# CHEBSB/PolarDecoding

Hardware: AMD Instinct MI355X
Metric: decoded frames/sec, N=1024 K=512 CA-SCL L=8 (higher is better)
Workload: dtype f64

## Files before the change

polardecoding_amd/csrc/scl_fast2.h:

```cpp
#pragma once
#include "fast2_lds.h"
#include "octet_bits.h"
#include "scl_fast.h"

namespace polar {

template <typename R>
struct Fast2Cfg {
    static constexpr int NLOG = 10, N = 1024, NW = 32, TOP = 9, HI = 8, L = 8;
    static constexpr int NA = 32;
    static constexpr int WAVES = 4;
    static constexpr int MIN_WAVES_PER_SIMD = sizeof(R) == 8 ? 3 : 4;
    static constexpr int NFA = HI - 3;
    static constexpr size_t sc_l8 = 0;
    static constexpr size_t sc_l7 = sc_l8 + 8 * 256;
    static constexpr size_t sc_l6 = sc_l7 + 8 * 128;
    static constexpr size_t sc_tl = sc_l6 + 8 * 64;
    static constexpr size_t scratch_cw = sc_tl + 512;
    static constexpr size_t scratch_elems = 2 * scratch_cw;
    static constexpr size_t off_lut = 0;
    static constexpr size_t off_frz = off_lut + ((Lut<R>::bytes + 15) / 16) * 16;
    static constexpr size_t off_msk = off_frz + 4 * NW;
    static constexpr size_t off_kth = off_msk + 4 * CRC_MASK_ROWS * NW;
    static constexpr size_t off_stair = off_kth + 256 * 8;
    static constexpr size_t shared_bytes = off_stair + ((Stair<R>::bytes + 15) / 16) * 16;
    static constexpr size_t off_bl = 0;
    static constexpr size_t off_cw = off_bl + 4 * fast2_lds::ROWS_WORDS;
    static constexpr size_t off_cd = off_cw + 4 * fast2_lds::ROWS_WORDS;
    static constexpr size_t off_ky = off_cd + sizeof(R) * 32;
    static constexpr size_t off_sg = off_ky + 128;
    static constexpr size_t per_wave = off_sg + sizeof(R) * 512;
    static constexpr size_t total = shared_bytes + WAVES * per_wave;
    static_assert(off_cw % 16 == 0 && off_cd % 16 == 0 && per_wave % 16 == 0 && shared_bytes % 16 == 0, "LDS regions are 16-byte aligned");
};
static_assert(3 * Fast2Cfg<double>::total <= 163840 && 4 * Fast2Cfg<float>::total <= 163840, "the pair kernel's LDS limits its occupancy");

template <int QP>
__device__ __forceinline__ double quadp(double x) { return quad_lanes<QP>(x); }
template <int QP>
__device__ __forceinline__ float quadp(float x) { return quad_lanes<QP>(x); }

template <bool FROM_Y>
struct Fast2Sigma { double sigma; };
template <>
struct Fast2Sigma<false> {};

template <typename R, typename IN, bool CRC_ON, bool FROM_Y>
struct Fast2Dec : Fast2Sigma<FROM_Y> {
    using C = Fast2Cfg<R>;
    static constexpr int N = C::N, NW = C::NW, TOP = C::TOP, HI = C::HI, L = 8, NFA = C::NFA;

    R A[C::NA];
    R a1;
    R bp_s, bp_d, bp_ts, bp_td;
    R PM;
    uint32_t ptr, bl0, fl;
    int logact;
    int p, c, pos, lane, gl;
    int own_addr, oth_addr;
    uint32_t pos0_mask;
    int cand_addr;
    Lut<R> lut;
    R *cand, *stg;
    uint32_t *blw, *curw, *keys;
    const unsigned char *kth;
    __amdgpu_buffer_rsrc_t rs_scr;
    __amdgpu_buffer_rsrc_t rs_in;
    unsigned cscr;
    unsigned csrc;
    static __device__ __forceinline__ __amdgpu_buffer_rsrc_t make_rsrc(const void *base, unsigned bytes)
    {
        return __builtin_amdgcn_make_buffer_rsrc(const_cast<void *>(base), 0, (int)bytes, 0x00020000);
    }
    typedef unsigned u2_t __attribute__((ext_vector_type(2)));
    static __device__ __forceinline__ double ld_buf(__amdgpu_buffer_rsrc_t r, unsigned eoff, double, int aux)
    {
        return aux ? __builtin_bit_cast(double, __builtin_amdgcn_raw_buffer_load_b64(r, eoff * 8u, 0, 16))
                   : __builtin_bit_cast(double, __builtin_amdgcn_raw_buffer_load_b64(r, eoff * 8u, 0, 0));
    }
    static __device__ __forceinline__ float ld_buf(__amdgpu_buffer_rsrc_t r, unsigned eoff, float, int aux)
    {
        return aux ? __builtin_bit_cast(float, __builtin_amdgcn_raw_buffer_load_b32(r, eoff * 4u, 0, 16))
                   : __builtin_bit_cast(float, __builtin_amdgcn_raw_buffer_load_b32(r, eoff * 4u, 0, 0));
    }
    static __device__ __forceinline__ void st_buf(__amdgpu_buffer_rsrc_t r, unsigned eoff, double v)
    {
        __builtin_amdgcn_raw_buffer_store_b64(__builtin_bit_cast(u2_t, v), r, eoff * 8u, 0, 0);
    }
    static __device__ __forceinline__ void st_buf(__amdgpu_buffer_rsrc_t r, unsigned eoff, float v)
    {
        __builtin_amdgcn_raw_buffer_store_b32(__builtin_bit_cast(unsigned, v), r, eoff * 4u, 0, 0);
    }
    struct SPtr {
        const Fast2Dec *d;
        unsigned off;
        struct Ref {
            const Fast2Dec *d;
            unsigned off;
            __device__ __forceinline__ void operator=(R v) const { st_buf(d->rs_scr, off, v); }
        };
        __device__ __forceinline__ SPtr operator+(int k) const { return SPtr{d, off + (unsigned)k}; }
        __device__ __forceinline__ Ref operator[](int k) const { return Ref{d, off + (unsigned)k}; }
    };
    static __device__ __forceinline__ R ld_sc(SPtr q) { return ld_buf(q.d->rs_scr, q.off, R(0), 1); }

    static __device__ __forceinline__ int row(int slot) { return fast2_lds::row(slot); }
    __device__ __forceinline__ int pa(int t) const { return (ptr >> (3 * (t - 4))) & 7; }
    __device__ __forceinline__ void set_pa(int t, int v) { ptr = (ptr & ~(7u << (3 * (t - 4)))) | ((uint32_t)v << (3 * (t - 4))); }
    __device__ __forceinline__ int pb(int t) const { return (ptr >> (3 * (NFA + t - 5))) & 7; }
    __device__ __forceinline__ void set_pb(int t, int v) { ptr = (ptr & ~(7u << (3 * (NFA + t - 5)))) | ((uint32_t)v << (3 * (NFA + t - 5))); }
    __device__ __forceinline__ R chk(R a, R b) const { return chk_lut1<R>(a, b, lut); }
    __device__ __forceinline__ R chks(R a, R b) const { return chk_lut1<R>(a, b, lut); }
    __device__ __forceinline__ R chv(int e) const
    {
        double v = (double)ld_buf(rs_in, csrc + (unsigned)e, IN(0), 0);
        if constexpr (FROM_Y) v = llr_from_y(v, this->sigma);
        return (R)v;
    }
    static __device__ __forceinline__ unsigned fresh(unsigned off)
    {
        __asm__ volatile("" : "+v"(off));
        return off;
    }
    __device__ __forceinline__ SPtr l8(int slot) const { return SPtr{this, fresh(cscr + (unsigned)(C::sc_l8 + slot * 256))}; }
    __device__ __forceinline__ SPtr l7(int slot) const { return SPtr{this, fresh(cscr + (unsigned)(C::sc_l7 + slot * 128))}; }
    __device__ __forceinline__ SPtr tls() const { return SPtr{this, fresh(cscr + (unsigned)C::sc_tl)}; }

    template <int T>
    __device__ __forceinline__ void f_reg()
    {
        constexpr int RO = (1 << T) / 4;
#pragma unroll
        for (int r = 0; r < RO; ++r) A[RO + r] = chk(A[2 * RO + r], A[3 * RO + r]);
        if constexpr (T >= 4) set_pa(T, p);
    }
    template <int T>
    __device__ __forceinline__ void g_reg()
    {
        constexpr int RO = (1 << T) / 4;
        const int sl = pa(T + 1) * 8 + gl;
        uint32_t w;
        if constexpr (T == 5) w = blw[row(pb(5)) + 1] >> pos;
        else w = bl0 >> (16 + pos);
#pragma unroll
        for (int r = 0; r < RO; ++r) {
            const R x = __shfl(A[2 * RO + r], sl), y = __shfl(A[3 * RO + r], sl);
            A[RO + r] = g_bit<R>(x, y, w, 4 * r);
        }
        set_pa(T, p);
    }
    __device__ __forceinline__ void g3()
    {
        const int sl = pa(4) * 8 + gl;
        const uint32_t w = bl0 >> (8 + pos);
#pragma unroll
        for (int r = 0; r < 2; ++r) {
            const R x = __shfl(A[4 + r], sl), y = __shfl(A[6 + r], sl);
            A[2 + r] = g_bit<R>(x, y, w, 4 * r);
        }
    }

    __device__ __forceinline__ void push_l6(R v)
    {
#pragma unroll
        for (int r = 16; r < 31; ++r) A[r] = A[r + 1];
        A[31] = v;
    }
    __device__ __forceinline__ void load_l6() { set_pa(6, p); }
    __device__ __forceinline__ R top_src(bool right, int idx, int q) const
    {
        const int seg = idx >> 4, within = idx & 15;
        const int e = 16 * q + within + 64 * (seg & 3) + 256 * (seg >> 2);
        return right ? chv(e) : ld_sc(tls() + e);
    }
    __device__ __forceinline__ void from_top(bool right, bool gstep)
    {
        vm_drain();
        const uint32_t *bt = blw + row(pb(TOP)) + 16;
        const uint32_t *bh = blw + row(pb(HI)) + 8;
        const SPtr o8 = l8(p), o7 = l7(p);
        const int w32 = (int)fresh((unsigned)(p * 4 + pos));
        const int nld = right ? 8 : 4;
        R *pre = A + 4;
#pragma unroll
        for (int m = 0; m < 8; ++m) pre[m] = (m < nld) ? top_src(right, w32 + 32 * m, 0) : R(0);
        for (int q = 0; q < 4; ++q) {
            lds_fence();
#pragma unroll
            for (int m = 0; m < 8; ++m)
                if (m < nld) stg[w32 + 32 * m] = pre[m];
            lds_fence();
            if (q < 3) {
#pragma unroll
                for (int m = 0; m < 8; ++m) pre[m] = (m < nld) ? top_src(right, w32 + 32 * m, q + 1) : R(0);
            }
#pragma unroll 1
            for (int i = 0; i < 4; ++i) {
                const int rr = 4 * q + i;
                const int e0 = pos + 4 * rr;
                const int sh = 4 * (rr & 7);
                const int wq = rr >> 3;
                const int wi = 4 * i + pos;
                R *v8 = A + 12;
#pragma unroll
                for (int k = 0; k < 4; ++k) {
                    const int e = e0 + 64 * k;
                    R x, y;
                    if (right) {
                        const uint32_t w0 = bt[2 * k + wq] >> pos, w1 = bt[8 + 2 * k + wq] >> pos;
                        x = g_bit<R>(stg[(k + 0) * 16 + wi], stg[(k + 8) * 16 + wi], w0, sh);
                        y = g_bit<R>(stg[(k + 4) * 16 + wi], stg[(k + 12) * 16 + wi], w1, sh);
                    } else {
                        x = stg[(k + 0) * 16 + wi];
                        y = stg[(k + 4) * 16 + wi];
                    }
                    if (gstep) v8[k] = g_bit<R>(x, y, bh[2 * k + wq] >> pos, sh);
                    else v8[k] = chk(x, y);
                    o8[e] = v8[k];
                }
                const R v70 = chk(v8[0], v8[2]), v71 = chk(v8[1], v8[3]);
                o7[e0] = v70;
                o7[e0 + 64] = v71;
                push_l6(chk(v70, v71));
            }
        }
        set_pa(8, p);
        set_pa(7, p);
        load_l6();
    }
    __device__ __forceinline__ void from_l8()
    {
        vm_drain();
        const SPtr s8 = l8(pa(8));
        const uint32_t *b7 = blw + row(pb(7)) + 4;
        const SPtr o7 = l7(p);
        constexpr int CP = sizeof(R) == 8 ? 2 : 4;
        for (int q = 0; q < 16 / CP; ++q) {
            R *in = A;
#pragma unroll
            for (int i = 0; i < CP; ++i) {
                const int e0 = pos + 4 * (CP * q + i);
#pragma unroll
                for (int k = 0; k < 4; ++k) in[4 * i + k] = ld_sc(s8 + e0 + 64 * k);
            }
#pragma unroll
            for (int i = 0; i < CP; ++i) {
                const int rr = CP * q + i;
                const int e0 = pos + 4 * rr;
                const int sh = 4 * (rr & 7);
                const int wq = rr >> 3;
                const R v70 = g_bit<R>(in[4 * i], in[4 * i + 2], b7[wq] >> pos, sh);
                const R v71 = g_bit<R>(in[4 * i + 1], in[4 * i + 3], b7[2 + wq] >> pos, sh);
                o7[e0] = v70;
                o7[e0 + 64] = v71;
                push_l6(chk(v70, v71));
            }
        }
        set_pa(7, p);
        load_l6();
    }
    __device__ __forceinline__ void from_l7()
    {
        vm_drain();
        const SPtr s7 = l7(pa(7)) + pos;
        const uint32_t *b6 = blw + row(pb(6)) + 2;
        const uint32_t w0 = b6[0] >> pos, w1 = b6[1] >> pos;
#pragma unroll
        for (int r = 0; r < 16; ++r) {
            const R x = ld_sc(s7 + 4 * r), y = ld_sc(s7 + 4 * r + 64);
            A[16 + r] = g_bit<R>(x, y, r < 8 ? w0 : w1, 4 * (r & 7));
        }
        set_pa(6, p);
    }

    __device__ __forceinline__ void octet_head(int o)
    {
        const int d = (o == 0) ? 10 : 3 + __builtin_ctz((unsigned)o);
        if (d >= 8) from_top(o >= N / 16, d == 8);
        else if (d == 7) from_l8();
        else if (d == 6) from_l7();
        else if (d == 5) g_reg<5>();
        else if (d == 4) g_reg<4>();
        else g3();
        if (d > 5) f_reg<5>();
        if (d > 4) f_reg<4>();
        if (d > 3) f_reg<3>();
    }
    __device__ __forceinline__ void octet_head_reg(int o)
    {
        const int d = 3 + __builtin_ctz((unsigned)o);
        if (d == 5) g_reg<5>();
        else if (d == 4) g_reg<4>();
        else g3();
        if (d > 4) f_reg<4>();
        if (d > 3) f_reg<3>();
    }

    template <int K>
    __device__ __forceinline__ void set_bit_k(int o, uint32_t bit)
    {
        if constexpr (K < 7) {
            bl0 |= bit << K;
        } else {
            const uint32_t c3 = octet_bits::level3((bl0 & 0x7Fu) | (bit << 7));
            bl0 &= ~0xFFu;
            set_bit7(o, c3);
        }
    }
    __device__ __forceinline__ void set_bit7(int o, uint32_t c3)
    {
        if ((o & 1) == 0) {
            bl0 = (bl0 & ~0xFF00u) | (c3 << 8);
            return;
        }
        const uint32_t c4 = (((bl0 >> 8) & 0xFFu) ^ c3) | (c3 << 8);
        if ((o & 2) == 0) {
            bl0 = (bl0 & 0xFFFFu) | (c4 << 16);
            return;
        }
        set_bit_lds(8 * o + 7, ((bl0 >> 16) ^ c4) | (c4 << 16));
    }
    __device__ __forceinline__ void set_bit_lds(int j, uint32_t cur)
    {
        const int own = (int)fresh((unsigned)row(p));
        lds_fence();
        if (pos == 0) curw[own] = cur;
        lds_fence();
        int t = 5;
        while (t < 10 && ((j >> t) & 1)) {
            const int nw = 1 << (t - 5);
            const int sb = pb(t);
            for (int w = pos; w < nw; w += 4) {
                const uint32_t cc = curw[own + w];
                const uint32_t l = blw[row(sb) + nw + w];
                curw[own + w] = l ^ cc;
                curw[own + w + nw] = cc;
            }
            lds_fence();
            ++t;
        }
        if (t < 10) {
            const int nw = 1 << (t - 5);
            for (int w = pos; w < nw; w += 4) blw[own + nw + w] = curw[own + w];
            set_pb(t, p);
            lds_fence();
        }
    }

    __device__ __forceinline__ uint32_t survivors(R c0, R c1)
    {
        lds_fence();
        if (pos == 0) {
            keys[2 * p] = metric_key(c0);
            keys[2 * p + 1] = metric_key(c1);
        }
        lds_fence();
        const unsigned char *kb = reinterpret_cast<const unsigned char *>(keys) - 64 * c;
        const uint32_t own = *reinterpret_cast<const uint32_t *>(kb + own_addr);
        const uint32_t oth = *reinterpret_cast<const uint32_t *>(kb + oth_addr);
        const uint32_t own1 = own + 1u;
        uint32_t acc = (oth - own1) >> 31;
        acc = __builtin_amdgcn_alignbit(acc, (uint32_t)dpp_i<0x121>((int)oth) - own1, 31);
        acc = __builtin_amdgcn_alignbit(acc, (uint32_t)dpp_i<0x122>((int)oth) - own1, 31);
        acc = __builtin_amdgcn_alignbit(acc, (uint32_t)dpp_i<0x123>((int)oth) - own1, 31);
        acc = __builtin_amdgcn_alignbit(acc, (uint32_t)dpp_i<0x124>((int)oth) - own1, 31);
        acc = __builtin_amdgcn_alignbit(acc, (uint32_t)dpp_i<0x125>((int)oth) - own1, 31);
        acc = __builtin_amdgcn_alignbit(acc, (uint32_t)dpp_i<0x126>((int)oth) - own1, 31);
        acc = __builtin_amdgcn_alignbit(acc, (uint32_t)dpp_i<0x127>((int)oth) - own1, 31);
        uint32_t cnt = __popc(acc);
        {
            auto r = __builtin_amdgcn_permlane16_swap(cnt, cnt, false, false);
            cnt = r[0] + r[1];
        }
        uint64_t b = __ballot(cnt <= (uint32_t)L);
        uint32_t m_a = (uint32_t)b & 0xFFFFu, m_b = (uint32_t)(b >> 32) & 0xFFFFu;
        if (sizeof(R) == 8 && (__popc(m_a) != L || __popc(m_b) != L)) {
            if (__popc(c ? m_b : m_a) != L) fl |= 0x4u;
            lds_fence();
            if (pos == 0) {
                cand[p] = c0;
                cand[8 + p] = c1;
            }
            lds_fence();
            const R *cb = reinterpret_cast<const R *>(reinterpret_cast<const unsigned char *>(cand) - (int)sizeof(R) * 16 * c);
            const R *mycand = reinterpret_cast<const R *>(reinterpret_cast<const unsigned char *>(cb) + cand_addr);
            const R mine = mycand[lane & 15];
            int n = 0;
#pragma unroll
            for (int m = 0; m < 16; ++m) n += (mycand[m] <= mine) ? 1 : 0;
            b = __ballot(n <= L);
            m_a = (uint32_t)b & 0xFFFFu;
            m_b = (uint32_t)(b >> 32) & 0xFFFFu;
        }
        return c ? m_b : m_a;
    }

    __device__ __forceinline__ bool trivial_prune(R cb, R cw) const
    {
        uint32_t mx = metric_key(cb) & pos0_mask;
        mx = max(mx, (uint32_t)dpp_i<0x128>((int)mx));
        {
            auto a = __builtin_amdgcn_permlane16_swap(mx, mx, false, false);
            mx = max(a[0], a[1]);
        }
        {
            auto a = __builtin_amdgcn_permlane32_swap(mx, mx, false, false);
            mx = max(a[0], a[1]);
        }
        return __ballot(mx >= (metric_key(cw) | ~pos0_mask)) == 0ull;
    }
    static __device__ __forceinline__ uint32_t sign_bit(double x) { return (uint32_t)__double2hiint(x) >> 31; }
    static __device__ __forceinline__ uint32_t sign_bit(float x) { return (uint32_t)__float_as_int(x) >> 31; }

    template <int K, bool FULL>
    __device__ __forceinline__ void decide(int o, bool frozen, R lam) { decide_t<K, FULL>(o, frozen, lam, lut.tabv(lam)); }
    template <int K, bool FULL>
    __device__ __forceinline__ void decide_t(int o, bool frozen, R lam, R tt)
    {
        if (frozen) {
            PM += tt + negmax(lam);
            set_bit_k<K>(o, 0u);
            return;
        }
        uint32_t bit;
        R pm;
        if (!FULL && logact < 3) {
            const R ph0 = tt + negmax(lam), ph1 = tt + posmax(lam);
            bit = (p >> logact) & 1;
            pm = PM + (bit ? ph1 : ph0);
            ++logact;
        } else {
            const uint32_t lneg = sign_bit(lam);
            const R cb = PM + tt, cw = PM + (tt + absr(lam));
            bit = (uint32_t)dpp_i<0x00>((int)lneg);
            pm = cb;
            if (!trivial_prune(cb, cw)) ranked<K>(lneg, cb, cw, bit, pm);
        }
        PM = pm;
        set_bit_k<K>(o, bit);
    }
    template <int K>
    __device__ __forceinline__ void ranked(uint32_t lneg, R cb, R cw, uint32_t &bit, R &pm)
    {
        const R c0 = lneg ? cw : cb, c1 = lneg ? cb : cw;
        const uint32_t mask = survivors(c0, c1);
        const uint32_t m0 = mask & 0xFFu, m1 = mask >> 8;
        const uint32_t m_both = m0 & m1, m_dead = ~(m0 | m1) & 0xFFu;
        if (__popc(mask) < L) fl |= 0x1u;
        const bool s0 = (m0 >> p) & 1, s1 = (m1 >> p) & 1;
        bit = (!s0 && s1) ? 1u : 0u;
        pm = bit ? c1 : c0;
        if (__ballot(m_dead != 0u) == 0ull) return;
        const bool dead = !s0 && !s1;
        const int myrank = __popc(m_dead & ((1u << p) - 1u));
        const bool refilled = dead && (myrank < __popc(m_both));
        const int src = (int)kth[m_both * 8 + myrank];
        const int sg = refilled ? src : p;
        const int sl = sg * 8 + gl;
        const R c1s = __shfl(c1, sl);
        ptr = __shfl(ptr, sl);
        bl0 = __shfl(bl0, sl);
        if constexpr ((K & 4) == 0) { A[2] = __shfl(A[2], sl); A[3] = __shfl(A[3], sl); }
        if constexpr ((K & 2) == 0) { A[1] = __shfl(A[1], sl); a1 = __shfl(a1, sl); }
        if constexpr ((K & 1) == 0) { bp_d = __shfl(bp_d, sl); bp_td = __shfl(bp_td, sl); }
        bit = refilled ? 1u : bit;
        pm = refilled ? c1s : pm;
    }

    __device__ __forceinline__ void frozen_prefix(int P, int nphi, bool regs, R &xl, R &yl)
    {
        const int w32 = p * 4 + pos, j0 = 8 * P;
        vm_drain();
        {
            const SPtr tl = tls();
            const SPtr o8 = l8(0), o7 = l7(0);
            R v8[8];
#pragma unroll
            for (int k = 0; k < 8; ++k) {
                const int e = w32 + 32 * k;
                v8[k] = chk(ld_sc(tl + e), ld_sc(tl + e + 256));
                o8[e] = v8[k];
            }
            lds_fence();
#pragma unroll
            for (int k = 0; k < 4; ++k) {
                const R v7 = chk(v8[k], v8[k + 4]);
                o7[w32 + 32 * k] = v7;
                stg[w32 + 32 * k] = v7;
            }
            set_pa(8, 0);
            set_pa(7, 0);
        }
        lds_fence();
#pragma unroll
        for (int t = 6; t >= 0; --t) {
            const int h = 1 << t;
            int idx[2];
            R x[2], y[2];
#pragma unroll
            for (int i = 0; i < 2; ++i) {
                const int b = w32 + 32 * i;
                idx[i] = ((b >> t) << (t + 1)) | (b & (h - 1));
                x[i] = stg[idx[i]];
                y[i] = stg[idx[i] + h];
            }
            if (t == 0) {
                xl = stg[126];
                yl = stg[127];
            }
            lds_fence();
#pragma unroll
            for (int i = 0; i < 2; ++i) {
                stg[idx[i]] = chk(x[i], y[i]);
                stg[idx[i] + h] = y[i] + x[i];
            }
            lds_fence();
            if (t >= 4 && regs) {
                const R *node = stg + ((j0 >> t) << t) + pos;
#pragma unroll
                for (int r = 0; r < h / 4; ++r) A[h / 4 + r] = node[4 * r];
            }
        }
#pragma unroll
        for (int k = 0; k < 4; ++k) {
            const R lam = stg[w32 + 32 * k];
            stg[128 + w32 + 32 * k] = lut.tabv(lam) + negmax(lam);
        }
        lds_fence();
        R pm = PM;
#pragma unroll 8
        for (int j = 0; j < nphi; ++j) pm += stg[128 + j];
        PM = pm;
        lds_fence();
    }

    __device__ __forceinline__ uint32_t fill_tail(uint32_t f2, R lam0, R xl, R yl)
    {
        uint32_t b0 = 0, b1 = 0;
        if (!(f2 & 1u)) {
            b0 = (p >> logact) & 1;
            ++logact;
        }
        PM += lut.tabv(lam0) + (b0 ? posmax(lam0) : negmax(lam0));
        const R lam1 = b0 ? -(xl - yl) : yl + xl;
        if (!(f2 & 2u)) {
            b1 = (p >> logact) & 1;
            ++logact;
        }
        PM += lut.tabv(lam1) + (b1 ? posmax(lam1) : negmax(lam1));
        return (b0 ? 0x55555555u : 0u) ^ (b1 ? 0xFFFFFFFFu : 0u);
    }
    __device__ __forceinline__ void fill_phase(int E, const uint32_t *frz, R xl, R yl)
    {
        const int w32 = (int)fresh((unsigned)(p * 4 + pos));
        const int qb = (p & 1) * 64;
        const uint32_t wv0 = fill_tail(frz[3] >> 30, stg[126], xl, yl);
        uint32_t wv1 = 0;
        lds_fence();
        blw[row(p) + 4 + pos] = wv0;
        lds_fence();
#pragma unroll 1
        for (int S = 128; S < E; S += 64) {
            vm_drain();
            const uint32_t wsel = S == 128 ? wv0 : wv1;
            uint32_t wq[2];
            wq[0] = (uint32_t)__shfl((int)wsel, gl) >> w32;
            wq[1] = (uint32_t)__shfl((int)wsel, 8 + gl) >> w32;
            if (S == 128) {
                const SPtr s8 = l8(0) + w32;
                R v8[8];
#pragma unroll
                for (int k = 0; k < 8; ++k) v8[k] = ld_sc(s8 + 32 * k);
#pragma unroll
                for (int q = 0; q < 2; ++q) {
                    const SPtr o7 = l7(q) + w32;
                    R v7[4];
#pragma unroll
                    for (int k = 0; k < 4; ++k) {
                        v7[k] = g_bit<R>(v8[k], v8[k + 4], wq[q], 0);
                        o7[32 * k] = v7[k];
                    }
                    stg[64 * q + w32] = chk(v7[0], v7[2]);
                    stg[64 * q + w32 + 32] = chk(v7[1], v7[3]);
                }
                set_pa(7, p & 1);
            } else {
#pragma unroll
                for (int q = 0; q < 2; ++q) {
                    const SPtr s7 = l7(q) + w32;
#pragma unroll
                    for (int i = 0; i < 2; ++i)
                        stg[64 * q + w32 + 32 * i] = g_bit<R>(ld_sc(s7 + 32 * i), ld_sc(s7 + 32 * i + 64), wq[q], 0);
                }
            }
            lds_fence();
#pragma unroll
            for (int t = 5; t >= 0; --t) {
                const int h = 1 << t;
                int idx[2];
                R x[2], y[2];
#pragma unroll
                for (int i = 0; i < 2; ++i) {
                    const int b = w32 + 32 * i;
                    idx[i] = ((b >> t) << (t + 1)) | (b & (h - 1));
                    x[i] = stg[idx[i]];
                    y[i] = stg[idx[i] + h];
                }
                if (t == 0) {
                    xl = stg[qb + 62];
                    yl = stg[qb + 63];
                }
                lds_fence();
#pragma unroll
                for (int i = 0; i < 2; ++i) {
                    stg[idx[i]] = chk(x[i], y[i]);
                    stg[idx[i] + h] = y[i] + x[i];
                }
                lds_fence();
            }
#pragma unroll
            for (int k = 0; k < 4; ++k) {
                const R lam = stg[w32 + 32 * k];
                stg[128 + w32 + 32 * k] = lut.tabv(lam) + negmax(lam);
            }
            lds_fence();
            R pm = PM;
#pragma unroll 2
            for (int j = 0; j < 62; ++j) pm += stg[128 + qb + j];
            PM = pm;
            const uint32_t wv = fill_tail(frz[(S + 62) >> 5] >> 30, stg[qb + 62], xl, yl);
            lds_fence();
            if (S == 128) {
                wv1 = wv;
                if (pos < 2) blw[row(p) + 2 + pos] = wv;
            } else {
                const uint32_t b = pos < 2 ? wv1 ^ wv : wv;
                blw[row(p) + 8 + pos] = wv0 ^ b;
                blw[row(p) + 12 + pos] = b;
            }
            lds_fence();
        }
    }

    template <bool FULL>
    __device__ __forceinline__ void octet_frozen_prefix(int o, bool last_frozen)
    {
        R xf = chks(A[2], A[3]), xg = A[3] + A[2];
        R yf = quadp<0x4E>(xf), yg = quadp<0x4E>(xg);
        {
            const R ff = chks(xf, yf), gf = xf + yf, fg = chks(xg, yg), gg = xg + yg;
            xf = (pos & 2) ? gf : ff;
            xg = (pos & 2) ? gg : fg;
        }
        yf = quadp<0xB1>(xf); yg = quadp<0xB1>(xg);
        R lf, lg;
        {
            const R ff = chks(xf, yf), gf = xf + yf, fg = chks(xg, yg), gg = xg + yg;
            lf = (pos & 1) ? gf : ff;
            lg = (pos & 1) ? gg : fg;
        }
        const R pf = lut.tabv(lf) + negmax(lf), pg = lut.tabv(lg) + negmax(lg);
        PM += pf;
        PM += quadp<0x55>(pf);
        PM += quadp<0xAA>(pf);
        PM += quadp<0xFF>(pf);
        PM += pg;
        PM += quadp<0x55>(pg);
        PM += quadp<0xAA>(pg);
        if (last_frozen) {
            PM += quadp<0xFF>(pg);
            set_bit7(o, 0u);
        } else {
            decide<7, FULL>(o, false, quadp<0xFF>(lg));
        }
    }

    struct ChkBp { R v, s, d, ts, td; };
    __device__ __forceinline__ ChkBp chk_bp(R x, R y) const
    {
        ChkBp r;
        r.s = x + y;
        r.d = x - y;
        r.ts = lut.tabv(r.s);
        r.td = lut.tabv(r.d);
        r.v = xor_sign(minabs(x, y), x, y) + (r.ts - r.td);
        return r;
    }
    static __device__ __forceinline__ R g_sel(R sum, R dif, uint32_t w, int sh)
    {
        const uint32_t m = (uint32_t)__builtin_amdgcn_sbfe((int)w, sh, 1);
        return Lut<R>::sel_mask(m, -dif, sum);
    }
    template <int K, bool FULL>
    __device__ __forceinline__ void leaf_pair(int o, uint32_t fm, R x1)
    {
        const ChkBp q = chk_bp(x1, quadp<0xB1>(x1));
        bp_d = q.d;
        bp_td = q.td;
        decide<K, FULL>(o, (fm >> K) & 1, q.v);
        const uint32_t m1 = (uint32_t)__builtin_amdgcn_sbfe((int)bl0, K, 1);
        decide_t<K + 1, FULL>(o, (fm >> (K + 1)) & 1, Lut<R>::sel_mask(m1, -bp_d, q.s), Lut<R>::sel_mask(m1, bp_td, q.ts));
    }
    template <bool FULL>
    __device__ __forceinline__ void octet(int o, uint32_t fm)
    {
        {
            const R s2 = A[2] + A[3], d2 = A[2] - A[3];
            const R v2 = xor_sign(minabs(A[2], A[3]), A[2], A[3]) + (lut.tabv(s2) - lut.tabv(d2));
            A[2] = s2;
            A[3] = d2;
            const R y2 = quadp<0x4E>(v2);
            const R s1 = v2 + y2, d1 = v2 - y2;
            const R v1 = xor_sign(minabs(v2, y2), v2, y2) + (lut.tabv(s1) - lut.tabv(d1));
            A[1] = s1;
            a1 = d1;
            leaf_pair<0, FULL>(o, fm, v1);
        }
        leaf_pair<2, FULL>(o, fm, g_sel(A[1], a1, octet_bits::level1_lo(bl0), pos));
        {
            const R v2 = g_sel(A[2], A[3], octet_bits::level2(bl0), pos);
            const R y2 = quadp<0x4E>(v2);
            const R s1 = v2 + y2, d1 = v2 - y2;
            const R v1 = xor_sign(minabs(v2, y2), v2, y2) + (lut.tabv(s1) - lut.tabv(d1));
            A[1] = s1;
            a1 = d1;
            leaf_pair<4, FULL>(o, fm, v1);
        }
        leaf_pair<6, FULL>(o, fm, g_sel(A[1], a1, octet_bits::level1_hi(bl0), pos));
    }
};

template <typename D, bool FULL>
__device__ __forceinline__ int octet_group(D &s, const uint32_t *frz, uint32_t &fword, int o)
{
    s.octet_head(o);
    for (;;) {
        if ((o & 3) == 0) fword = frz[o >> 2];
        const uint32_t fm = (fword >> (8 * (o & 3))) & 0xFFu;
        if ((fm & 0x7Fu) != 0x7Fu) s.template octet<FULL>(o, fm);
        else s.template octet_frozen_prefix<FULL>(o, fm == 0xFFu);
        ++o;
        if ((o & 7) == 0) break;
        s.octet_head_reg(o);
    }
    return o;
}

template <typename R, typename IN, bool CRC_ON, bool FROM_Y>
__device__ __forceinline__ void scl_fast2_body(const SclParams &P)
{
    using D = Fast2Dec<R, IN, CRC_ON, FROM_Y>;
    using C = Fast2Cfg<R>;
    constexpr int N = C::N, NW = C::NW, L = 8;
    extern __shared__ __attribute__((aligned(16))) unsigned char smem[];
    const int wave = __builtin_amdgcn_readfirstlane(threadIdx.x >> 6);
    unsigned char *base = smem + C::shared_bytes + (size_t)wave * C::per_wave;
    uint32_t *frz = reinterpret_cast<uint32_t *>(smem + C::off_frz);
    uint32_t *msk = reinterpret_cast<uint32_t *>(smem + C::off_msk);
    unsigned char *kth = smem + C::off_kth;

    Lut<R>::build(smem + C::off_lut, threadIdx.x, blockDim.x);
    for (int i = threadIdx.x; i < NW; i += blockDim.x) frz[i] = P.frozen[i];
    if (CRC_ON)
        for (int i = threadIdx.x; i < CRC_MASK_ROWS * NW; i += blockDim.x)
            msk[i] = P.crc_mask[(i & ~(NW - 1)) + ((i >> 3) & 3) + 4 * (i & 7)];
    for (int i = threadIdx.x; i < 256 * 8; i += blockDim.x) {
        int m = i >> 3, k = i & 7, idx = 0, seen = 0;
        for (int b = 0; b < 8; ++b)
            if ((m >> b) & 1) {
                if (seen == k) idx = b;
                ++seen;
            }
        kth[i] = (unsigned char)idx;
    }
    __syncthreads();

    D s;
    s.lane = threadIdx.x & 63;
    s.p = s.lane >> 3;
    s.c = (s.lane >> 2) & 1;
    s.pos = s.lane & 3;
    s.pos0_mask = s.pos == 0 ? 0xFFFFFFFFu : 0u;
    s.gl = s.lane & 7;
    s.lut.bind(smem + C::off_lut);
    s.kth = kth;
    s.blw = reinterpret_cast<uint32_t *>(base + C::off_bl) + fast2_lds::cw_base(1) * s.c;
    s.curw = reinterpret_cast<uint32_t *>(base + C::off_cw) + fast2_lds::cw_base(1) * s.c;
    s.cand = reinterpret_cast<R *>(base + C::off_cd) + s.c * 16;
    s.keys = reinterpret_cast<uint32_t *>(base + C::off_ky) + s.c * 16;
    s.stg = reinterpret_cast<R *>(base + C::off_sg) + s.c * 256;
    if constexpr (FROM_Y) s.sigma = P.sigma;
    {
        const int i = s.lane & 15, row = s.lane >> 4, cwr = row >> 1, h = row & 1;
        const int jj = (i + 8 * h) & 15;
        s.own_addr = 64 * cwr + 4 * (2 * (i & 7) + (i >> 3));
        s.oth_addr = 64 * cwr + 4 * (2 * (jj & 7) + (jj >> 3));
        s.cand_addr = (int)sizeof(R) * 16 * cwr;
    }
    const int lane = s.lane, p = s.p, c = s.c, pos = s.pos;
    const int wave_global = blockIdx.x * C::WAVES + wave;
    const int waves_total = gridDim.x * C::WAVES;
    R *scr_wave = reinterpret_cast<R *>(P.scratch) + (size_t)wave_global * C::scratch_elems;
    s.rs_scr = D::make_rsrc(scr_wave, (unsigned)(C::scratch_elems * sizeof(R)));
    s.cscr = (unsigned)c * (unsigned)C::scratch_cw;

    int lead = 0;
    while (lead < 15 && ((frz[lead >> 2] >> (8 * (lead & 3))) & 0xFFu) == 0xFFu) ++lead;
    lead = __builtin_amdgcn_readfirstlane(lead);
    const int E = P.fill_end;

    for (int pair = wave_global; 2 * pair < P.B;) {
        const int frame_raw = 2 * pair + c;
        const bool live = frame_raw < P.B;
        const int frame = live ? frame_raw : P.B - 1;
        s.rs_in = D::make_rsrc(reinterpret_cast<const IN *>(P.in) + (size_t)(2 * pair) * N, (unsigned)(2 * N * sizeof(IN)));
        s.csrc = (unsigned)(frame - 2 * pair) * (unsigned)N;
        {
            const auto t = s.tls();
            const int w = p * 4 + pos;
#pragma unroll 2
            for (int e = w; e < N / 2; e += 32) t[e] = s.chk(s.chv(e), s.chv(e + N / 2));
        }
#pragma unroll
        for (int j = 0; j < NW / 4; ++j) s.blw[D::row(p) + pos + 4 * j] = 0;
        lds_fence();

        s.PM = R(0);
        s.ptr = 0;
        for (int t = 4; t <= 8; ++t) s.set_pa(t, p);
        for (int t = 5; t <= 9; ++t) s.set_pb(t, p);
        s.bl0 = 0;
        s.a1 = R(0);
#pragma unroll
        for (int r = 0; r < C::NA; ++r) s.A[r] = R(0);
        s.fl = 0;
        s.logact = 0;
        uint32_t fword = 0;

        int o_first = 0;
        if (E > 0 || lead > 0) {
            R xl, yl;
            s.frozen_prefix(E > 0 ? 15 : lead, E > 0 ? 126 : 8 * lead, E == 0, xl, yl);
            o_first = lead;
            if (E > 0) {
                s.fill_phase(E, frz, xl, yl);
                o_first = E >> 3;
            }
            fword = frz[o_first >> 2];
        }
        int o = o_first;
#pragma unroll 1
        while (o < N / 8 && s.logact < 3) o = octet_group<D, false>(s, frz, fword, o);
        while (o < N / 8) o = octet_group<D, true>(s, frz, fword, o);

        bool pass = false;
        if constexpr (CRC_ON) {
            lds_fence();
            uint32_t x[8];
#pragma unroll
            for (int j = 0; j < 8; ++j) x[j] = s.curw[D::row(p) + pos + 4 * j];
            typedef uint32_t u4_t __attribute__((ext_vector_type(4)));
            const u4_t *mk = reinterpret_cast<const u4_t *>(msk + 8 * pos);
            const int rows = (P.crc_r + 3) & ~3;
            uint32_t rem = 0;
#pragma unroll 1
            for (int i = 0; i < rows; i += 4) {
#pragma unroll
                for (int k = 0; k < 4; ++k) {
                    const u4_t a = mk[(i + k) * (NW / 4)], b = mk[(i + k) * (NW / 4) + 1];
                    const uint32_t acc = (x[0] & a.x) ^ (x[1] & a.y) ^ (x[2] & a.z) ^ (x[3] & a.w) ^ (x[4] & b.x) ^
                                         (x[5] & b.y) ^ (x[6] & b.z) ^ (x[7] & b.w);
                    rem |= (uint32_t)(__popc(acc) & 1) << (i + k);
                }
            }
            rem ^= (uint32_t)dpp_i<0xB1>((int)rem);
            rem ^= (uint32_t)dpp_i<0x4E>((int)rem);
            pass = rem == 0u;
        }
        const uint64_t bp_ = __ballot(pass && pos == 0);
        const uint64_t cwmask = 0x0101010101010101ull << (4 * c);
        const bool any = (bp_ & cwmask) != 0ull;
        int best = -1;
        R best_pm = R(0);
        for (int q = 0; q < L; ++q) {
            const R pq = __shfl(s.PM, q * 8 + 4 * c);
            const int okq = __shfl((int)(any ? pass : true), q * 8 + 4 * c);
            if (okq && (best < 0 || pq < best_pm)) {
                best = q;
                best_pm = pq;
            }
        }
        uint32_t fl = s.fl;
        if (any) fl |= 0x2u;
        lds_fence();
        {
            const int w = p * 4 + pos;
            uint32_t x = s.curw[D::row(best) + w];
            x = polar_word_transform(x);
#pragma unroll
            for (int hw = 1; hw < NW; hw <<= 1) {
                const int wo = w ^ hw;
                const uint32_t ov = __shfl(x, (wo >> 2) * 8 + 4 * c + (wo & 3));
                if (!(w & hw)) x ^= ov;
            }
            if (live) P.out_bits[(size_t)frame * NW + w] = x;
        }
        if (live && p == 0 && pos == 0) {
            if (P.pm) P.pm[frame] = (double)best_pm;
            if (P.flags) P.flags[frame] = fl;
        }
        lds_fence();
        pair = next_job_wave(P.queue, pair, waves_total, (P.B + 1) >> 1);
    }
}

template <typename R, typename IN, bool CRC_ON>
__global__ __launch_bounds__(256, (Fast2Cfg<R>::MIN_WAVES_PER_SIMD)) void k_scl_fast2(SclParams P)
{
    scl_fast2_body<R, IN, CRC_ON, false>(P);
}
template <typename R, typename IN, bool CRC_ON>
__global__ __launch_bounds__(256, (Fast2Cfg<R>::MIN_WAVES_PER_SIMD)) void k_scl_fast2_y(SclParams P)
{
    scl_fast2_body<R, IN, CRC_ON, true>(P);
}

}
```

Measured before the change: 15.36 million.

## Permute f64 scratch layout so paired LLRs use 128-bit buffer loads/stores

Introduces a permutation sigma on the level-7/8 scratch rows for f64. Each lane's two passes (elements e and e+4) become adjacent and 16-byte aligned. from_l8 and from_l7 then read and write pairs with single b128 buffer loads and stores instead of two b64 accesses, which cuts the number of memory instructions. All other producers and consumers of these rows are remapped through sigma to stay consistent, with static_asserts checking bijection and alignment. The risk is a missed access site left in the old layout, and changed per-lane coalescing patterns.

```diff
diff --git a/polardecoding_amd/csrc/fast2_scratch.h b/polardecoding_amd/csrc/fast2_scratch.h
--- /dev/null
+++ b/polardecoding_amd/csrc/fast2_scratch.h
@@ -0,0 +1,70 @@
+#pragma once
+
+namespace polar {
+namespace fast2_scratch {
+
+constexpr int ROW8 = 256, ROW7 = 128, SLOTS = 8;
+constexpr int ROW6 = 64, TL = 512;
+constexpr int SC_L8 = 0;
+constexpr int SC_L7 = SC_L8 + SLOTS * ROW8;
+constexpr int SC_L6 = SC_L7 + SLOTS * ROW7;
+constexpr int SC_TL = SC_L6 + SLOTS * ROW6;
+constexpr int SCRATCH_CW = SC_TL + TL;
+
+constexpr unsigned sigma(unsigned e) { return (e & ~7u) | ((e & 3u) << 1) | ((e >> 2) & 1u); }
+constexpr unsigned pair_at(unsigned pos, unsigned m) { return 8u * m + 2u * pos; }
+
+constexpr bool bijection(int n)
+{
+    for (int s = 0; s < n; ++s) {
+        int hits = 0;
+        for (int e = 0; e < n; ++e) hits += sigma((unsigned)e) == (unsigned)s;
+        if (hits != 1) return false;
+    }
+    return true;
+}
+constexpr bool pairs_adjacent_and_aligned(int n, int elem_bytes)
+{
+    for (unsigned pos = 0; pos < 4; ++pos)
+        for (unsigned m = 0; 8 * m < (unsigned)n; ++m) {
+            const unsigned a = sigma(pos + 8 * m), b = sigma(pos + 8 * m + 4);
+            if (b != a + 1 || a % 2 || a != pair_at(pos, m)) return false;
+            if ((a * (unsigned)elem_bytes) % (2u * (unsigned)elem_bytes)) return false;
+        }
+    return true;
+}
+constexpr bool path_covers_a_block(int n)
+{
+    for (unsigned m = 0; 8 * m < (unsigned)n; ++m) {
+        unsigned seen = 0;
+        for (unsigned pos = 0; pos < 4; ++pos)
+            for (unsigned h = 0; h < 2; ++h) {
+                const unsigned s = sigma(pos + 8 * m + 4 * h);
+                if (s < 8 * m || s >= 8 * m + 8) return false;
+                seen |= 1u << (s - 8 * m);
+            }
+        if (seen != 0xFFu) return false;
+    }
+    return true;
+}
+constexpr bool strides_pass_through(int n)
+{
+    for (int e = 0; e < 8; ++e)
+        for (int k = 0; 8 * k + e < n; ++k)
+            if (sigma((unsigned)(e + 8 * k)) != sigma((unsigned)e) + 8u * (unsigned)k) return false;
+    return true;
+}
+constexpr bool rows_pair_aligned()
+{
+    return SC_L8 % 2 == 0 && SC_L7 % 2 == 0 && SCRATCH_CW % 2 == 0 && ROW8 % 2 == 0 && ROW7 % 2 == 0;
+}
+static_assert(bijection(ROW7) && bijection(ROW8), "sigma is not a bijection on a row");
+static_assert(pairs_adjacent_and_aligned(ROW7, 8) && pairs_adjacent_and_aligned(ROW8, 8) && pairs_adjacent_and_aligned(ROW7, 4) &&
+                  pairs_adjacent_and_aligned(ROW8, 4),
+              "a lane's two passes are not one aligned pair");
+static_assert(path_covers_a_block(ROW7) && path_covers_a_block(ROW8), "a path's four lanes do not cover 8 consecutive elements");
+static_assert(strides_pass_through(ROW7) && strides_pass_through(ROW8), "sigma(e + 8k) != sigma(e) + 8k");
+static_assert(rows_pair_aligned(), "a row does not start at a multiple of two elements");
+
+}
+}
diff --git a/polardecoding_amd/csrc/scl_fast2.h b/polardecoding_amd/csrc/scl_fast2.h
--- a/polardecoding_amd/csrc/scl_fast2.h
+++ b/polardecoding_amd/csrc/scl_fast2.h
@@ -1,5 +1,6 @@
 #pragma once
 #include "fast2_lds.h"
+#include "fast2_scratch.h"
 #include "octet_bits.h"
 #include "scl_fast.h"
 
@@ -12,12 +13,13 @@
     static constexpr int WAVES = 4;
     static constexpr int MIN_WAVES_PER_SIMD = sizeof(R) == 8 ? 3 : 4;
     static constexpr int NFA = HI - 3;
-    static constexpr size_t sc_l8 = 0;
-    static constexpr size_t sc_l7 = sc_l8 + 8 * 256;
-    static constexpr size_t sc_l6 = sc_l7 + 8 * 128;
-    static constexpr size_t sc_tl = sc_l6 + 8 * 64;
-    static constexpr size_t scratch_cw = sc_tl + 512;
+    static constexpr size_t sc_l8 = fast2_scratch::SC_L8;
+    static constexpr size_t sc_l7 = fast2_scratch::SC_L7;
+    static constexpr size_t sc_l6 = fast2_scratch::SC_L6;
+    static constexpr size_t sc_tl = fast2_scratch::SC_TL;
+    static constexpr size_t scratch_cw = fast2_scratch::SCRATCH_CW;
     static constexpr size_t scratch_elems = 2 * scratch_cw;
+    static constexpr bool PAIRED = sizeof(R) == 8;
     static constexpr size_t off_lut = 0;
     static constexpr size_t off_frz = off_lut + ((Lut<R>::bytes + 15) / 16) * 16;
     static constexpr size_t off_msk = off_frz + 4 * NW;
@@ -91,6 +93,21 @@
     {
         __builtin_amdgcn_raw_buffer_store_b32(__builtin_bit_cast(unsigned, v), r, eoff * 4u, 0, 0);
     }
+    typedef unsigned u4_t __attribute__((ext_vector_type(4)));
+    struct R2 {
+        R a, b;
+    };
+    static __device__ __forceinline__ R2 ld_buf2(__amdgpu_buffer_rsrc_t r, unsigned eoff, int aux)
+    {
+        static_assert(sizeof(R2) == 16, "paired accesses are for f64");
+        return aux ? __builtin_bit_cast(R2, __builtin_amdgcn_raw_buffer_load_b128(r, eoff * 8u, 0, 16))
+                   : __builtin_bit_cast(R2, __builtin_amdgcn_raw_buffer_load_b128(r, eoff * 8u, 0, 0));
+    }
+    static __device__ __forceinline__ void st_buf2(__amdgpu_buffer_rsrc_t r, unsigned eoff, R2 v)
+    {
+        static_assert(sizeof(R2) == 16, "paired accesses are for f64");
+        __builtin_amdgcn_raw_buffer_store_b128(__builtin_bit_cast(u4_t, v), r, eoff * 8u, 0, 0);
+    }
     struct SPtr {
         const Fast2Dec *d;
         unsigned off;
@@ -103,6 +120,21 @@
         __device__ __forceinline__ Ref operator[](int k) const { return Ref{d, off + (unsigned)k}; }
     };
     static __device__ __forceinline__ R ld_sc(SPtr q) { return ld_buf(q.d->rs_scr, q.off, R(0), 1); }
+    static __device__ __forceinline__ int sg(int e) { return C::PAIRED ? (int)fast2_scratch::sigma((unsigned)e) : e; }
+    static __device__ __forceinline__ int sg2(int pos, int m) { return C::PAIRED ? (int)fast2_scratch::pair_at((unsigned)pos, (unsigned)m) : pos + 8 * m; }
+    static __device__ __forceinline__ R2 ld_sc2(SPtr q)
+    {
+        if constexpr (C::PAIRED) return ld_buf2(q.d->rs_scr, q.off, 1);
+        else return R2{ld_sc(q), ld_sc(q + sg(4))};
+    }
+    static __device__ __forceinline__ void st_sc2(SPtr q, R a, R b)
+    {
+        if constexpr (C::PAIRED) st_buf2(q.d->rs_scr, q.off, R2{a, b});
+        else {
+            q[0] = a;
+            q[sg(4)] = b;
+        }
+    }
 
     static __device__ __forceinline__ int row(int slot) { return fast2_lds::row(slot); }
     __device__ __forceinline__ int pa(int t) const { return (ptr >> (3 * (t - 4))) & 7; }
@@ -197,14 +229,13 @@
 #pragma unroll 1
             for (int i = 0; i < 4; ++i) {
                 const int rr = 4 * q + i;
-                const int e0 = pos + 4 * rr;
+                const int s0 = sg(pos + 4 * rr);
                 const int sh = 4 * (rr & 7);
                 const int wq = rr >> 3;
                 const int wi = 4 * i + pos;
                 R *v8 = A + 12;
 #pragma unroll
                 for (int k = 0; k < 4; ++k) {
-                    const int e = e0 + 64 * k;
                     R x, y;
                     if (right) {
                         const uint32_t w0 = bt[2 * k + wq] >> pos, w1 = bt[8 + 2 * k + wq] >> pos;
@@ -216,11 +247,11 @@
                     }
                     if (gstep) v8[k] = g_bit<R>(x, y, bh[2 * k + wq] >> pos, sh);
                     else v8[k] = chk(x, y);
-                    o8[e] = v8[k];
+                    o8[s0 + 64 * k] = v8[k];
                 }
                 const R v70 = chk(v8[0], v8[2]), v71 = chk(v8[1], v8[3]);
-                o7[e0] = v70;
-                o7[e0 + 64] = v71;
+                o7[s0] = v70;
+                o7[s0 + 64] = v71;
                 push_l6(chk(v70, v71));
             }
         }
@@ -235,25 +266,36 @@
         const uint32_t *b7 = blw + row(pb(7)) + 4;
         const SPtr o7 = l7(p);
         constexpr int CP = sizeof(R) == 8 ? 2 : 4;
+        static_assert(CP % 2 == 0 && 4 * CP <= 16, "a chunk is whole pairs of passes and fits the dead registers");
         for (int q = 0; q < 16 / CP; ++q) {
             R *in = A;
 #pragma unroll
-            for (int i = 0; i < CP; ++i) {
-                const int e0 = pos + 4 * (CP * q + i);
-#pragma unroll
-                for (int k = 0; k < 4; ++k) in[4 * i + k] = ld_sc(s8 + e0 + 64 * k);
-            }
-#pragma unroll
-            for (int i = 0; i < CP; ++i) {
-                const int rr = CP * q + i;
-                const int e0 = pos + 4 * rr;
-                const int sh = 4 * (rr & 7);
-                const int wq = rr >> 3;
-                const R v70 = g_bit<R>(in[4 * i], in[4 * i + 2], b7[wq] >> pos, sh);
-                const R v71 = g_bit<R>(in[4 * i + 1], in[4 * i + 3], b7[2 + wq] >> pos, sh);
-                o7[e0] = v70;
-                o7[e0 + 64] = v71;
-                push_l6(chk(v70, v71));
+            for (int j = 0; j < CP / 2; ++j) {
+                const int m = CP / 2 * q + j;
+#pragma unroll
+                for (int k = 0; k < 4; ++k) {
+                    const R2 v = ld_sc2(s8 + sg2(pos, m) + 64 * k);
+                    in[8 * j + k] = v.a;
+                    in[8 * j + 4 + k] = v.b;
+                }
+            }
+#pragma unroll
+            for (int j = 0; j < CP / 2; ++j) {
+                const int m = CP / 2 * q + j;
+                R v70[2], v71[2];
+#pragma unroll
+                for (int h = 0; h < 2; ++h) {
+                    const int i = 2 * j + h;
+                    const int rr = CP * q + i;
+                    const int sh = 4 * (rr & 7);
+                    const int wq = rr >> 3;
+                    v70[h] = g_bit<R>(in[4 * i], in[4 * i + 2], b7[wq] >> pos, sh);
+                    v71[h] = g_bit<R>(in[4 * i + 1], in[4 * i + 3], b7[2 + wq] >> pos, sh);
+                }
+                st_sc2(o7 + sg2(pos, m), v70[0], v70[1]);
+                st_sc2(o7 + sg2(pos, m) + 64, v71[0], v71[1]);
+                push_l6(chk(v70[0], v71[0]));
+                push_l6(chk(v70[1], v71[1]));
             }
         }
         set_pa(7, p);
@@ -262,13 +304,15 @@
     __device__ __forceinline__ void from_l7()
     {
         vm_drain();
-        const SPtr s7 = l7(pa(7)) + pos;
+        const SPtr s7 = l7(pa(7));
         const uint32_t *b6 = blw + row(pb(6)) + 2;
         const uint32_t w0 = b6[0] >> pos, w1 = b6[1] >> pos;
 #pragma unroll
-        for (int r = 0; r < 16; ++r) {
-            const R x = ld_sc(s7 + 4 * r), y = ld_sc(s7 + 4 * r + 64);
-            A[16 + r] = g_bit<R>(x, y, r < 8 ? w0 : w1, 4 * (r & 7));
+        for (int m = 0; m < 8; ++m) {
+            const R2 x = ld_sc2(s7 + sg2(pos, m)), y = ld_sc2(s7 + sg2(pos, m) + 64);
+            const int r = 2 * m;
+            A[16 + r] = g_bit<R>(x.a, y.a, r < 8 ? w0 : w1, 4 * (r & 7));
+            A[17 + r] = g_bit<R>(x.b, y.b, r < 8 ? w0 : w1, 4 * ((r + 1) & 7));
         }
         set_pa(6, p);
     }
@@ -473,19 +517,19 @@
         vm_drain();
         {
             const SPtr tl = tls();
-            const SPtr o8 = l8(0), o7 = l7(0);
+            const SPtr o8 = l8(0) + sg(w32), o7 = l7(0) + sg(w32);
             R v8[8];
 #pragma unroll
             for (int k = 0; k < 8; ++k) {
                 const int e = w32 + 32 * k;
                 v8[k] = chk(ld_sc(tl + e), ld_sc(tl + e + 256));
-                o8[e] = v8[k];
+                o8[32 * k] = v8[k];
             }
             lds_fence();
 #pragma unroll
             for (int k = 0; k < 4; ++k) {
                 const R v7 = chk(v8[k], v8[k + 4]);
-                o7[w32 + 32 * k] = v7;
+                o7[32 * k] = v7;
                 stg[w32 + 32 * k] = v7;
             }
             set_pa(8, 0);
@@ -567,13 +611,13 @@
             wq[0] = (uint32_t)__shfl((int)wsel, gl) >> w32;
             wq[1] = (uint32_t)__shfl((int)wsel, 8 + gl) >> w32;
             if (S == 128) {
-                const SPtr s8 = l8(0) + w32;
+                const SPtr s8 = l8(0) + sg(w32);
                 R v8[8];
 #pragma unroll
                 for (int k = 0; k < 8; ++k) v8[k] = ld_sc(s8 + 32 * k);
 #pragma unroll
                 for (int q = 0; q < 2; ++q) {
-                    const SPtr o7 = l7(q) + w32;
+                    const SPtr o7 = l7(q) + sg(w32);
                     R v7[4];
 #pragma unroll
                     for (int k = 0; k < 4; ++k) {
@@ -587,7 +631,7 @@
             } else {
 #pragma unroll
                 for (int q = 0; q < 2; ++q) {
-                    const SPtr s7 = l7(q) + w32;
+                    const SPtr s7 = l7(q) + sg(w32);
 #pragma unroll
                     for (int i = 0; i < 2; ++i)
                         stg[64 * q + w32 + 32 * i] = g_bit<R>(ld_sc(s7 + 32 * i), ld_sc(s7 + 32 * i + 64), wq[q], 0);
```

After: 15.60 million, median of 6. 1.02x the previous value.
